# IvanPopov/video-flow-ml

Measured on AMD Instinct MI355X. Metric: flow-fields/sec @1080p seq5 MOF_sintel, higher is better.
Workload: dtype mixed (per-layer MFMA count, f32 accumulate): {"corr": 1, "update_block.encoder.convf1": 1, "update_block.encoder.convf2": 1, "update_block.gru.convq1.iter": "2a", "update_block.gru.convzr1.iter": 1, "update_block.gru.convzr2.iter": 1, "update_block.mask.0": 1, "update_block.mask.2": 1, "update_bloc

## Files before the change

### video-flow-ml_amd/vfml/csrc/enc_conv.hip

```cpp
#include "conv_split_common.h"

namespace {

constexpr int EC_C = 64;
constexpr int EC_TH = 4, EC_TW = 32;
constexpr int EC_PR = EC_TH + 2, EC_PW = EC_TW + 2;
constexpr int EC_PIX = 272;
constexpr int EC_PATCH = EC_PR * EC_PW * EC_PIX;
constexpr int EC_VLD = EC_C + 4;
constexpr int EC_LDS = EC_PATCH;
constexpr int EC_K = 9 * EC_C;
constexpr int EC_NS = EC_K / 32;
static_assert(EC_TH * EC_TW * EC_VLD * 4 <= EC_PATCH, "the result tile fits where the patch was");

struct EncConvArgs {
  const char* in;
  const _Float16* whi; const _Float16* wlo;
  const float* bias;
  float* out; int ldo;
  double* stats_part;
  int ld_in, n, H, W, tiles_x, tiles_y;
  float w_inv;
};

__global__ __launch_bounds__(256, 2) void enc_conv3x3_c64_kernel(const EncConvArgs a) {
  extern __shared__ __attribute__((aligned(16))) char smem[];
  float* sV = reinterpret_cast<float*>(smem);

  const int t = threadIdx.x, lane = t & 63;
  const int wave = __builtin_amdgcn_readfirstlane(t >> 6);
  const int r4 = lane & 15, u4 = lane >> 4;
  const int tiles_img = a.tiles_x * a.tiles_y;
  const int total = a.n * tiles_img;

  h16x8 bh[EC_NS], bl[EC_NS];
  static_for<EC_NS>([&](auto sc) {
    constexpr int s = decltype(sc)::value;
    bh[s] = *reinterpret_cast<const h16x8*>(a.whi + (16 * wave + r4) * EC_K + s * 32 + u4 * 8);
    bl[s] = *reinterpret_cast<const h16x8*>(a.wlo + (16 * wave + r4) * EC_K + s * 32 + u4 * 8);
  });
  f32x4 bias4 = {0.f, 0.f, 0.f, 0.f};
  if (a.bias) bias4 = *reinterpret_cast<const f32x4*>(a.bias + 16 * wave + 4 * u4);

  for (int tile = blockIdx.x; tile < total; tile += gridDim.x) {
    const int img = tile / tiles_img, tl = tile - img * tiles_img;
    const int ty = tl / a.tiles_x, tx = tl - ty * a.tiles_x;
    const int oy0 = ty * EC_TH, ox0 = tx * EC_TW;

    constexpr int NPC = EC_PR * EC_PW * 16;
    constexpr int NPT = (NPC + 255) / 256;
    const __amdgpu_buffer_rsrc_t rin = __builtin_amdgcn_make_buffer_rsrc(
        const_cast<char*>(a.in) + (int64_t)img * a.H * a.W * a.ld_in * 4, 0, a.H * a.W * a.ld_in * 4, 0x00020000);
    u32x4 pv[NPT];
    static_for<NPT>([&](auto qc) {
      constexpr int q = decltype(qc)::value;
      const int c = min(t + 256 * q, NPC - 1);
      const int p = c >> 4, piece = c & 15;
      const int py = p / EC_PW, px = p - py * EC_PW;
      const int iy = oy0 - 1 + py, ix = ox0 - 1 + px;
      const bool ok = (unsigned)iy < (unsigned)a.H && (unsigned)ix < (unsigned)a.W;
      pv[q] = bload16(rin, ok ? ((iy * a.W + ix) * a.ld_in) * 4 + piece * 16 : (int)0x80000000);
    });
    __syncthreads();
    static_for<NPT>([&](auto qc) {
      constexpr int q = decltype(qc)::value;
      const int c = t + 256 * q;
      if (c < NPC) *reinterpret_cast<u32x4*>(smem + (c >> 4) * EC_PIX + (c & 15) * 16) = pv[q];
    });
    __syncthreads();

    f32x4 acc[8];
#pragma unroll
    for (int m = 0; m < 8; ++m) acc[m] = f32x4{0.f, 0.f, 0.f, 0.f};
    const char* al = smem + r4 * EC_PIX + u4 * 32;
    static_for<2>([&](auto hc) {
      constexpr int mh = decltype(hc)::value;
      static_for<EC_NS>([&](auto sc) {
        constexpr int s = decltype(sc)::value;
        constexpr int cb = s / 9, ky = (s % 9) / 3, kx = s % 3;
#pragma unroll
        for (int mm = 0; mm < 4; ++mm) {
          const int m = 4 * mh + mm;
          const char* p = al + (((m >> 1) + ky) * EC_PW + 16 * (m & 1) + kx) * EC_PIX + cb * 128;
          const h16x8 ah = *reinterpret_cast<const h16x8*>(p);
          const h16x8 alo = *reinterpret_cast<const h16x8*>(p + 16);
          acc[m] = __builtin_amdgcn_mfma_f32_16x16x32_f16(bh[s], ah, acc[m], 0, 0, 0);
          acc[m] = __builtin_amdgcn_mfma_f32_16x16x32_f16(bl[s], ah, acc[m], 0, 0, 0);
          acc[m] = __builtin_amdgcn_mfma_f32_16x16x32_f16(bh[s], alo, acc[m], 0, 0, 0);
        }
        if constexpr (s % 3 == 2) __builtin_amdgcn_sched_barrier(0);
      });
      __builtin_amdgcn_sched_barrier(0);
    });

    __syncthreads();
#pragma unroll
    for (int m = 0; m < 8; ++m) {
      f32x4 v;
#pragma unroll
      for (int e = 0; e < 4; ++e) v[e] = acc[m][e] * a.w_inv + bias4[e];
      const int row = m >> 1, col = 16 * (m & 1) + r4;
      const int oy = oy0 + row, ox = ox0 + col;
      *reinterpret_cast<f32x4*>(&sV[(row * EC_TW + col) * EC_VLD + 16 * wave + 4 * u4]) = v;
      if (oy < a.H && ox < a.W)
        *reinterpret_cast<f32x4*>(a.out + (((int64_t)img * a.H + oy) * a.W + ox) * a.ldo + 16 * wave + 4 * u4) = v;
    }
    if (a.stats_part) {
      __syncthreads();
      const int row = t >> 6, ch = t & 63;
      const int oy = oy0 + row;
      if (oy < a.H) {
        double s1 = 0.0, s2 = 0.0;
        for (int x = 0; x < EC_TW; ++x) {
          float f = sV[(row * EC_TW + x) * EC_VLD + ch], g;
          asm("v_mov_b32 %0, %1" : "=v"(g) : "v"(f));
          const double v = (double)g;
          s1 += v;
          s2 += v * v;
        }
        const int64_t chunk = (((int64_t)img * a.H + oy) * a.W + ox0) >> 5;
        double* o = a.stats_part + (chunk * EC_C + ch) * 2;
        o[0] = s1;
        o[1] = s2;
      }
    }
  }
}

}

extern "C" int vfml_conv3x3_c64(const float* in, int ld_in, int n, int h, int w, const void* w_hi, const void* w_lo, int kp,
                                float w_scale, const float* bias, float* out, int ldo, double* stats_part, void* stream) {
  VFML_REQUIRE(in && w_hi && w_lo && out && n > 0 && h > 0 && w > 0, "vfml_conv3x3_c64: bad argument");
  VFML_REQUIRE(w % EC_TW == 0, "vfml_conv3x3_c64: the image width must be a multiple of %d (got %d)", EC_TW, w);
  VFML_REQUIRE(kp == EC_K && w_scale > 0.f, "vfml_conv3x3_c64: weight planes [64][%d] (VFML_KORDER_CBLOCK), got row pitch %d", EC_K, kp);
  VFML_REQUIRE((reinterpret_cast<uintptr_t>(in) & 31u) == 0 && ld_in >= EC_C && ld_in % 8 == 0 && vfml_aligned16(w_hi) &&
                   vfml_aligned16(w_lo) && vfml_aligned16(bias) && vfml_aligned16(out) && ldo >= EC_C && ldo % 4 == 0 &&
                   (reinterpret_cast<uintptr_t>(stats_part) & 7u) == 0,
               "vfml_conv3x3_c64: a 32-byte aligned split-row input (ld_in %% 8 == 0), 16-byte aligned weights / bias / output "
               "(ldo %% 4 == 0)");
  EncConvArgs a;
  a.in = reinterpret_cast<const char*>(in); a.ld_in = ld_in;
  a.whi = reinterpret_cast<const _Float16*>(w_hi); a.wlo = reinterpret_cast<const _Float16*>(w_lo);
  a.bias = bias; a.out = out; a.ldo = ldo; a.stats_part = stats_part;
  a.n = n; a.H = h; a.W = w; a.tiles_x = w / EC_TW; a.tiles_y = (h + EC_TH - 1) / EC_TH;
  a.w_inv = 1.0f / w_scale;
  const int64_t total = (int64_t)n * a.tiles_x * a.tiles_y;
  VFML_REQUIRE(total < (1ll << 31) && (int64_t)h * w * ld_in * 4 < (1ll << 31), "vfml_conv3x3_c64: an image of the input must stay below 2 GiB");
  const int grid = (int)(total < 512 ? total : 512);
  hipLaunchKernelGGL(enc_conv3x3_c64_kernel, dim3(grid), dim3(256), EC_LDS, reinterpret_cast<hipStream_t>(stream), a);
  return vfml_check_launch("vfml_conv3x3_c64");
}
```

### video-flow-ml_amd/vfml/csrc/flow_half.hip

```cpp
#include "conv_split_common.h"

namespace {

constexpr int FH_TH = 4, FH_TW = 30;
constexpr int FH_FR = FH_TH + 2, FH_FW = 32;
constexpr int FH_PR = FH_FR + 6, FH_PW = 40;
constexpr int FH_PATCH = FH_PR * FH_PW * 8;
constexpr int FH_F1PIX = 272;
constexpr int FH_F1 = FH_FR * FH_FW * FH_F1PIX;
constexpr int FH_LDS = FH_PATCH + FH_F1;
constexpr int FH_K1 = 7 * 32, FH_K2 = 9 * 128;
constexpr int FH_RING = 12;

struct FlowHalfArgs {
  const f32x4* flow;
  const _Float16* w1;
  const _Float16* w2;
  const float* b1; const float* b2;
  float* out; int ld_out;
  int n, h, w, tiles_x, tiles_y;
  float w1_inv, w2_inv;
};

__global__ __launch_bounds__(256, 2) void flow_half_kernel(const FlowHalfArgs a) {
  extern __shared__ __attribute__((aligned(16))) char smem[];
  char* patch = smem;
  char* f1 = smem + FH_PATCH;

  const int t = threadIdx.x, lane = t & 63;
  const int wave = __builtin_amdgcn_readfirstlane(t >> 6);
  const int tiles = a.tiles_x * a.tiles_y;
  const int img = blockIdx.x / tiles, tl = blockIdx.x - img * tiles;
  const int ty = tl / a.tiles_x, tx = tl - ty * a.tiles_x;
  const int oy0 = ty * FH_TH, ox0 = tx * FH_TW;
  const int r4 = lane & 15, u4 = lane >> 4;

  const f32x4* src = a.flow + (int64_t)img * a.h * a.w;
  constexpr int NPP = (FH_PR * FH_PW + 255) / 256;
  f32x4 pv[NPP];
  bool pok[NPP];
  static_for<NPP>([&](auto qc) {
    constexpr int q = decltype(qc)::value;
    const int p = min(t + 256 * q, FH_PR * FH_PW - 1);
    const int py = p / FH_PW, px = p - py * FH_PW;
    const int iy = oy0 - 4 + py, ix = ox0 - 4 + px;
    pok[q] = (unsigned)iy < (unsigned)a.h && (unsigned)ix < (unsigned)a.w;
    pv[q] = src[(int64_t)min(max(iy, 0), a.h - 1) * a.w + min(max(ix, 0), a.w - 1)];
  });
  h16x8 w1f[7][2];
  static_for<7>([&](auto kc) {
    constexpr int ky = decltype(kc)::value;
#pragma unroll
    for (int j = 0; j < 2; ++j)
      w1f[ky][j] = *reinterpret_cast<const h16x8*>(a.w1 + (32 * wave + 16 * j + r4) * FH_K1 + ky * 32 + u4 * 8);
  });
  f32x4 b1v[2];
#pragma unroll
  for (int j = 0; j < 2; ++j) b1v[j] = *reinterpret_cast<const f32x4*>(a.b1 + 32 * wave + 16 * j + 4 * u4);
  static_for<NPP>([&](auto qc) {
    constexpr int q = decltype(qc)::value;
    const int p = t + 256 * q;
    if (p < FH_PR * FH_PW) {
      const f32x4 v = pok[q] ? pv[q] : f32x4{0.f, 0.f, 0.f, 0.f};
      const h16x2 h0 = {(_Float16)v[0], (_Float16)v[1]}, h1 = {(_Float16)v[2], (_Float16)v[3]};
      *reinterpret_cast<uint2*>(patch + p * 8) = uint2{__builtin_bit_cast(unsigned, h0), __builtin_bit_cast(unsigned, h1)};
    }
  });
  __syncthreads();

  static_for<FH_FR>([&](auto rc) {
    constexpr int fy = decltype(rc)::value;
    f32x4 acc[2][2];
#pragma unroll
    for (int s = 0; s < 2; ++s)
#pragma unroll
      for (int j = 0; j < 2; ++j) acc[s][j] = f32x4{0.f, 0.f, 0.f, 0.f};
    static_for<7>([&](auto kc) {
      constexpr int ky = decltype(kc)::value;
#pragma unroll
      for (int s = 0; s < 2; ++s) {
        const char* p = patch + (((fy + ky) * FH_PW) + 16 * s + r4 + 2 * u4) * 8;
        const uint2 lo = *reinterpret_cast<const uint2*>(p), hi = *reinterpret_cast<const uint2*>(p + 8);
        const h16x8 av = __builtin_bit_cast(h16x8, u32x4{lo.x, lo.y, hi.x, hi.y});
#pragma unroll
        for (int j = 0; j < 2; ++j) acc[s][j] = __builtin_amdgcn_mfma_f32_16x16x32_f16(w1f[ky][j], av, acc[s][j], 0, 0, 0);
      }
    });
    const int iy = oy0 - 1 + fy;
#pragma unroll
    for (int s = 0; s < 2; ++s) {
      const int ix = ox0 - 1 + 16 * s + r4;
      const bool inside = (unsigned)iy < (unsigned)a.h && (unsigned)ix < (unsigned)a.w;
#pragma unroll
      for (int j = 0; j < 2; ++j) {
        f32x4 v;
#pragma unroll
        for (int e = 0; e < 4; ++e) v[e] = inside ? fmaxf(acc[s][j][e] * a.w1_inv + b1v[j][e], 0.f) : 0.f;
        const h16x2 h0 = {(_Float16)v[0], (_Float16)v[1]}, h1 = {(_Float16)v[2], (_Float16)v[3]};
        *reinterpret_cast<uint2*>(f1 + (fy * FH_FW + 16 * s + r4) * FH_F1PIX + (32 * wave + 16 * j + 4 * u4) * 2) =
            uint2{__builtin_bit_cast(unsigned, h0), __builtin_bit_cast(unsigned, h1)};
      }
    }
  });
  __syncthreads();

  f32x4 acc[8];
#pragma unroll
  for (int m = 0; m < 8; ++m) acc[m] = f32x4{0.f, 0.f, 0.f, 0.f};
  const _Float16* w2row = a.w2 + (16 * wave + r4) * FH_K2 + u4 * 8;
  constexpr int NS = FH_K2 / 32;
  h16x8 ring[FH_RING];
  static_for<FH_RING>([&](auto sc) {
    constexpr int s = decltype(sc)::value;
    ring[s] = *reinterpret_cast<const h16x8*>(w2row + (s >> 1) * 64 + (s & 1) * 32);
  });
  const char* f1l = f1 + r4 * FH_F1PIX + u4 * 16;
  static_for<NS>([&](auto sc) {
    constexpr int s = decltype(sc)::value;
    constexpr int cb = s / 18, tap = (s % 18) / 2, half = s & 1, ky = tap / 3, kx = tap % 3;
    const h16x8 bv = ring[s % FH_RING];
    if constexpr (s + FH_RING < NS) {
      constexpr int n = s + FH_RING;
      ring[s % FH_RING] = *reinterpret_cast<const h16x8*>(w2row + (n >> 1) * 64 + (n & 1) * 32);
    }
#pragma unroll
    for (int m = 0; m < 8; ++m) {
      const h16x8 av = *reinterpret_cast<const h16x8*>(f1l + (((m >> 1) + ky) * FH_FW + ((m & 1) ? 14 : 0) + kx) * FH_F1PIX +
                                                        (cb * 64 + half * 32) * 2);
      acc[m] = __builtin_amdgcn_mfma_f32_16x16x32_f16(bv, av, acc[m], 0, 0, 0);
    }
  });

  const f32x4 b2v = *reinterpret_cast<const f32x4*>(a.b2 + 16 * wave + 4 * u4);
#pragma unroll
  for (int m = 0; m < 8; ++m) {
    const int oy = oy0 + (m >> 1), col = ((m & 1) ? 14 : 0) + r4;
    const int ox = ox0 + col;
    if (oy >= a.h || ox >= a.w || ((m & 1) && r4 < 2)) continue;
    f32x4 v;
#pragma unroll
    for (int e = 0; e < 4; ++e) v[e] = fmaxf(acc[m][e] * a.w2_inv + b2v[e], 0.f);
    vfml_h16x2 h0, h1, l0, l1;
    vfml_split2(v[0], v[1], h0, l0);
    vfml_split2(v[2], v[3], h1, l1);
    char* u = reinterpret_cast<char*>(a.out + ((int64_t)img * a.h * a.w + (int64_t)oy * a.w + ox) * a.ld_out + 8 * (2 * wave + (u4 >> 1))) +
              (u4 & 1) * 8;
    *reinterpret_cast<uint2*>(u) = uint2{__builtin_bit_cast(unsigned, h0), __builtin_bit_cast(unsigned, h1)};
    *reinterpret_cast<uint2*>(u + 16) = uint2{__builtin_bit_cast(unsigned, l0), __builtin_bit_cast(unsigned, l1)};
  }
}

}

extern "C" int vfml_flow_half(const float* flow, int n, int h, int w, const void* w1_hi, int kp1, float w1_scale, const float* b1,
                              const void* w2_hi, int kp2, float w2_scale, const float* b2, float* out, int ld_out, void* stream) {
  VFML_REQUIRE(flow && w1_hi && w2_hi && b1 && b2 && out && n > 0 && h > 0 && w > 0, "vfml_flow_half: bad argument");
  VFML_REQUIRE(kp1 == FH_K1 && kp2 == FH_K2, "vfml_flow_half: weight planes [128][%d] (vfml_flow_rows7 layout) and [64][%d] "
               "(VFML_KORDER_CBLOCK64), got row pitches %d / %d", FH_K1, FH_K2, kp1, kp2);
  VFML_REQUIRE(w1_scale > 0.f && w2_scale > 0.f, "vfml_flow_half: weight scales must be positive");
  VFML_REQUIRE(vfml_aligned16(flow) && vfml_aligned16(w1_hi) && vfml_aligned16(w2_hi) && vfml_aligned16(b1) && vfml_aligned16(b2) &&
                   (reinterpret_cast<uintptr_t>(out) & 31u) == 0 && ld_out >= 64 && ld_out % 8 == 0,
               "vfml_flow_half: 16-byte aligned operands, a 32-byte aligned split-row output with ld_out %% 8 == 0");
  FlowHalfArgs a;
  a.flow = reinterpret_cast<const f32x4*>(flow);
  a.w1 = reinterpret_cast<const _Float16*>(w1_hi); a.w2 = reinterpret_cast<const _Float16*>(w2_hi);
  a.b1 = b1; a.b2 = b2; a.out = out; a.ld_out = ld_out;
  a.n = n; a.h = h; a.w = w;
  a.tiles_x = (w + FH_TW - 1) / FH_TW; a.tiles_y = (h + FH_TH - 1) / FH_TH;
  a.w1_inv = 1.0f / w1_scale; a.w2_inv = 1.0f / w2_scale;
  const int64_t grid = (int64_t)n * a.tiles_x * a.tiles_y;
  VFML_REQUIRE(grid < (1ll << 31), "vfml_flow_half: too many tiles");
  if (const int rc = vfml_lds_cap(reinterpret_cast<const void*>(&flow_half_kernel), FH_LDS, "vfml_flow_half")) return rc;
  hipLaunchKernelGGL(flow_half_kernel, dim3((unsigned)grid), dim3(256), FH_LDS, reinterpret_cast<hipStream_t>(stream), a);
  return vfml_check_launch("vfml_flow_half");
}
```

Before: 46.26.

## Reuse LDS activation fragments across ky taps in encoder and flow convolutions

Both 3x3 conv kernels now walk patch rows instead of output rows. Each LDS activation fragment (patch row, kx, channel block) is loaded once into a double-buffered register set and fed to every output row it contributes to across the three ky taps. This cuts LDS reads by up to roughly 3x and prefetches the next fragment while the MFMAs run. In flow_half the rolling weight ring is replaced by all conv2 weights held in registers, with the first block loaded early, which raises VGPR pressure and risks spills or lower occupancy.

```diff
diff --git a/video-flow-ml_amd/vfml/csrc/enc_conv.hip b/video-flow-ml_amd/vfml/csrc/enc_conv.hip
--- a/video-flow-ml_amd/vfml/csrc/enc_conv.hip
+++ b/video-flow-ml_amd/vfml/csrc/enc_conv.hip
@@ -52,9 +52,11 @@
     const __amdgpu_buffer_rsrc_t rin = __builtin_amdgcn_make_buffer_rsrc(
         const_cast<char*>(a.in) + (int64_t)img * a.H * a.W * a.ld_in * 4, 0, a.H * a.W * a.ld_in * 4, 0x00020000);
     u32x4 pv[NPT];
+    int tl0 = t, tl1 = t;
+    asm volatile("" : "+v"(tl0), "+v"(tl1));
     static_for<NPT>([&](auto qc) {
       constexpr int q = decltype(qc)::value;
-      const int c = min(t + 256 * q, NPC - 1);
+      const int c = min(tl0 + 256 * q, NPC - 1);
       const int p = c >> 4, piece = c & 15;
       const int py = p / EC_PW, px = p - py * EC_PW;
       const int iy = oy0 - 1 + py, ix = ox0 - 1 + px;
@@ -64,7 +66,7 @@
     __syncthreads();
     static_for<NPT>([&](auto qc) {
       constexpr int q = decltype(qc)::value;
-      const int c = t + 256 * q;
+      const int c = tl1 + 256 * q;
       if (c < NPC) *reinterpret_cast<u32x4*>(smem + (c >> 4) * EC_PIX + (c & 15) * 16) = pv[q];
     });
     __syncthreads();
@@ -73,22 +75,38 @@
 #pragma unroll
     for (int m = 0; m < 8; ++m) acc[m] = f32x4{0.f, 0.f, 0.f, 0.f};
     const char* al = smem + r4 * EC_PIX + u4 * 32;
-    static_for<2>([&](auto hc) {
-      constexpr int mh = decltype(hc)::value;
-      static_for<EC_NS>([&](auto sc) {
-        constexpr int s = decltype(sc)::value;
-        constexpr int cb = s / 9, ky = (s % 9) / 3, kx = s % 3;
+    constexpr int NW = 2 * EC_PR * 3;
+    h16x8 fa[2][2][2];
+    auto frag = [&](auto ic) {
+      constexpr int i = decltype(ic)::value;
+      constexpr int cb = i / (3 * EC_PR), pr = (i / 3) % EC_PR, kx = i % 3;
 #pragma unroll
-        for (int mm = 0; mm < 4; ++mm) {
-          const int m = 4 * mh + mm;
-          const char* p = al + (((m >> 1) + ky) * EC_PW + 16 * (m & 1) + kx) * EC_PIX + cb * 128;
-          const h16x8 ah = *reinterpret_cast<const h16x8*>(p);
-          const h16x8 alo = *reinterpret_cast<const h16x8*>(p + 16);
-          acc[m] = __builtin_amdgcn_mfma_f32_16x16x32_f16(bh[s], ah, acc[m], 0, 0, 0);
-          acc[m] = __builtin_amdgcn_mfma_f32_16x16x32_f16(bl[s], ah, acc[m], 0, 0, 0);
-          acc[m] = __builtin_amdgcn_mfma_f32_16x16x32_f16(bh[s], alo, acc[m], 0, 0, 0);
-        }
-        if constexpr (s % 3 == 2) __builtin_amdgcn_sched_barrier(0);
+      for (int hf = 0; hf < 2; ++hf) {
+        const char* p = al + (pr * EC_PW + 16 * hf + kx) * EC_PIX + cb * 128;
+        fa[i & 1][hf][0] = *reinterpret_cast<const h16x8*>(p);
+        fa[i & 1][hf][1] = *reinterpret_cast<const h16x8*>(p + 16);
+      }
+    };
+    frag(std::integral_constant<int, 0>{});
+    static_for<NW>([&](auto ic) {
+      constexpr int i = decltype(ic)::value;
+      constexpr int cb = i / (3 * EC_PR), pr = (i / 3) % EC_PR, kx = i % 3;
+      if constexpr (i + 1 < NW) {
+        frag(std::integral_constant<int, i + 1>{});
+        __builtin_amdgcn_sched_barrier(0);
+      }
+      static_for<3>([&](auto jc) {
+        constexpr int j = decltype(jc)::value;
+        static_for<3>([&](auto kc) {
+          constexpr int ky = decltype(kc)::value, r = pr - ky;
+          if constexpr (r >= 0 && r < EC_TH) {
+            constexpr int s = cb * 9 + ky * 3 + kx;
+#pragma unroll
+            for (int hf = 0; hf < 2; ++hf)
+              acc[2 * r + hf] = __builtin_amdgcn_mfma_f32_16x16x32_f16(j == 1 ? bl[s] : bh[s], fa[i & 1][hf][j == 2 ? 1 : 0],
+                                                                       acc[2 * r + hf], 0, 0, 0);
+          }
+        });
       });
       __builtin_amdgcn_sched_barrier(0);
     });
diff --git a/video-flow-ml_amd/vfml/csrc/flow_half.hip b/video-flow-ml_amd/vfml/csrc/flow_half.hip
--- a/video-flow-ml_amd/vfml/csrc/flow_half.hip
+++ b/video-flow-ml_amd/vfml/csrc/flow_half.hip
@@ -10,7 +10,6 @@
 constexpr int FH_F1 = FH_FR * FH_FW * FH_F1PIX;
 constexpr int FH_LDS = FH_PATCH + FH_F1;
 constexpr int FH_K1 = 7 * 32, FH_K2 = 9 * 128;
-constexpr int FH_RING = 12;
 
 struct FlowHalfArgs {
   const f32x4* flow;
@@ -54,6 +53,16 @@
     for (int j = 0; j < 2; ++j)
       w1f[ky][j] = *reinterpret_cast<const h16x8*>(a.w1 + (32 * wave + 16 * j + r4) * FH_K1 + ky * 32 + u4 * 8);
   });
+  const _Float16* w2row = a.w2 + (16 * wave + r4) * FH_K2 + u4 * 8;
+  h16x8 w2f[2][9][2];
+  auto load_w2 = [&](auto cc) {
+    constexpr int cb = decltype(cc)::value;
+    static_for<18>([&](auto sc) {
+      constexpr int s = decltype(sc)::value;
+      w2f[cb][s >> 1][s & 1] = *reinterpret_cast<const h16x8*>(w2row + cb * 576 + (s >> 1) * 64 + (s & 1) * 32);
+    });
+  };
+  load_w2(std::integral_constant<int, 0>{});
   f32x4 b1v[2];
 #pragma unroll
   for (int j = 0; j < 2; ++j) b1v[j] = *reinterpret_cast<const f32x4*>(a.b1 + 32 * wave + 16 * j + 4 * u4);
@@ -107,28 +116,41 @@
   f32x4 acc[8];
 #pragma unroll
   for (int m = 0; m < 8; ++m) acc[m] = f32x4{0.f, 0.f, 0.f, 0.f};
-  const _Float16* w2row = a.w2 + (16 * wave + r4) * FH_K2 + u4 * 8;
-  constexpr int NS = FH_K2 / 32;
-  h16x8 ring[FH_RING];
-  static_for<FH_RING>([&](auto sc) {
-    constexpr int s = decltype(sc)::value;
-    ring[s] = *reinterpret_cast<const h16x8*>(w2row + (s >> 1) * 64 + (s & 1) * 32);
-  });
+  load_w2(std::integral_constant<int, 1>{});
   const char* f1l = f1 + r4 * FH_F1PIX + u4 * 16;
-  static_for<NS>([&](auto sc) {
-    constexpr int s = decltype(sc)::value;
-    constexpr int cb = s / 18, tap = (s % 18) / 2, half = s & 1, ky = tap / 3, kx = tap % 3;
-    const h16x8 bv = ring[s % FH_RING];
-    if constexpr (s + FH_RING < NS) {
-      constexpr int n = s + FH_RING;
-      ring[s % FH_RING] = *reinterpret_cast<const h16x8*>(w2row + (n >> 1) * 64 + (n & 1) * 32);
+  constexpr int NW = 2 * FH_FR * 3;
+  h16x8 fa[2][2][2];
+  auto frag = [&](auto ic) {
+    constexpr int i = decltype(ic)::value;
+    constexpr int cb = i / (3 * FH_FR), pr = (i / 3) % FH_FR, kx = i % 3;
+#pragma unroll
+    for (int hf = 0; hf < 2; ++hf)
+#pragma unroll
+      for (int half = 0; half < 2; ++half)
+        fa[i & 1][hf][half] = *reinterpret_cast<const h16x8*>(f1l + (pr * FH_FW + (hf ? 14 : 0) + kx) * FH_F1PIX +
+                                                                (cb * 64 + half * 32) * 2);
+  };
+  frag(std::integral_constant<int, 0>{});
+  static_for<NW>([&](auto ic) {
+    constexpr int i = decltype(ic)::value;
+    constexpr int cb = i / (3 * FH_FR), pr = (i / 3) % FH_FR, kx = i % 3;
+    if constexpr (i + 1 < NW) {
+      frag(std::integral_constant<int, i + 1>{});
+      __builtin_amdgcn_sched_barrier(0);
     }
+    static_for<2>([&](auto hc) {
+      constexpr int half = decltype(hc)::value;
+      static_for<3>([&](auto kc) {
+        constexpr int ky = decltype(kc)::value, r = pr - ky;
+        if constexpr (r >= 0 && r < FH_TH) {
 #pragma unroll
-    for (int m = 0; m < 8; ++m) {
-      const h16x8 av = *reinterpret_cast<const h16x8*>(f1l + (((m >> 1) + ky) * FH_FW + ((m & 1) ? 14 : 0) + kx) * FH_F1PIX +
-                                                        (cb * 64 + half * 32) * 2);
-      acc[m] = __builtin_amdgcn_mfma_f32_16x16x32_f16(bv, av, acc[m], 0, 0, 0);
-    }
+          for (int hf = 0; hf < 2; ++hf)
+            acc[2 * r + hf] = __builtin_amdgcn_mfma_f32_16x16x32_f16(w2f[cb][ky * 3 + kx][half], fa[i & 1][hf][half],
+                                                                     acc[2 * r + hf], 0, 0, 0);
+        }
+      });
+    });
+    __builtin_amdgcn_sched_barrier(0);
   });
 
   const f32x4 b2v = *reinterpret_cast<const f32x4*>(a.b2 + 16 * wave + 4 * u4);
```

After: 46.25. About the same (-0.0%).
